# tencent-ailab/V-Express

Hardware: AMD Instinct MI355X
Metric: decoded frames/sec at 512x512, 25 DDIM steps (higher is better)
Workload: dtype bf16; 1 GPU; 512x512, 16 frames (1 window(s) of 16, overlap 4), 25 DDIM steps, CFG 3.5, random-init UNet3D + ReferenceNet banks + sd-vae-ft-mse decode; frames=16, windows=1, parallelism=window x CFG-half units over 1 GPU(s)

## Files before the change

### v-express_amd/csrc/vx_attn.hip

```cpp
#include "vx_common.h"
#include <stdio.h>
#include "../../include/vexpress_hip.h"

#include <stdlib.h>

#include <type_traits>

namespace {

struct AttnParams {
  const bf16_t* q; int ldq;
  const bf16_t* k; int ldk;
  const bf16_t* vt; int vt_pitch;
  bf16_t* out; int ldo;
  int batch, heads, n_q, n_kv, d, q_per_kv;
  float c;
  const float* kmax;
};

__device__ __forceinline__ int k_lds_off(int slab, int key, int grp) {
  return slab * 4096 + key * 64 + ((grp ^ ((0 - (key >> 2)) & 3)) << 4);
}
__device__ __forceinline__ int v_lds_off(int row, int chunk) { return row * 128 + ((chunk ^ ((row >> 1) & 7)) << 4); }

// ... 798 lines not shown
    best = fmaxf(best, ss);
  }
  red[threadIdx.x] = best;
  __syncthreads();
  for (int s = 128; s > 0; s >>= 1) {
    if ((int)threadIdx.x < s) red[threadIdx.x] = fmaxf(red[threadIdx.x], red[threadIdx.x + s]);
    __syncthreads();
  }
  if (threadIdx.x == 0) out[bh] = sqrtf(red[0]);
}

constexpr int KNM8_KEYS = 256;
__global__ __launch_bounds__(256) void key_norm_max8_kernel(const bf16_t* __restrict__ k, int ldk, int n_kv, int d,
                                                            float* __restrict__ out) {
  __shared__ float red[4][8];
  const int b = blockIdx.y, key0 = blockIdx.x * KNM8_KEYS;
  const int lane = threadIdx.x & 63, wave = threadIdx.x >> 6, h = lane & 7;
  const bf16_t* base = k + (size_t)b * n_kv * ldk + h * d;
  const int chunks = d >> 3;
  float best = 0.f;
  for (int kk = wave * 8 + (lane >> 3); kk < KNM8_KEYS; kk += 32) {
    const int key = min(key0 + kk, n_kv - 1);
    const bf16_t* row = base + (size_t)key * ldk;
    float ss = 0.f;
    for (int c = 0; c < chunks; ++c) {
      float f[8];
      unpack_bf16x8(*reinterpret_cast<const uint4*>(row + 8 * c), f);
#pragma unroll
      for (int e = 0; e < 8; ++e) ss = fmaf(f[e], f[e], ss);
    }
    best = fmaxf(best, ss);
  }
  best = fmaxf(best, __shfl_xor(best, 8, 64));
  best = fmaxf(best, __shfl_xor(best, 16, 64));
  best = fmaxf(best, __shfl_xor(best, 32, 64));
  if (lane < 8) red[wave][lane] = best;
  __syncthreads();
  if (threadIdx.x < 8) {
    const float m = fmaxf(fmaxf(red[0][threadIdx.x], red[1][threadIdx.x]), fmaxf(red[2][threadIdx.x], red[3][threadIdx.x]));
    atomicMax(reinterpret_cast<unsigned int*>(out) + b * 8 + threadIdx.x, __float_as_uint(sqrtf(m)));
  }
}

int attention_impl(const void* q, int ldq, const void* k, int ldk, const void* vt, int vt_pitch, void* out, int ldo,
                   int batch, int heads, int n_q, int n_kv, int head_dim, int q_per_kv, float scale,
                   const float* key_norm_max, hipStream_t stream);

}

int vx_attn3_variant();
int vx_attn3_launch(const void* q, int ldq, const void* k, int ldk, const void* vt, int vt_pitch, void* out, int ldo,
                    int batch, int heads, int n_q, int n_kv, int q_per_kv, float c, const float* kmax,
                    hipStream_t stream);

extern "C" int vx_key_norm_max(const void* k, int ldk, int kv_batches, int heads, int n_kv, int head_dim, float* out,
                               void* stream) {
  VX_REQUIRE(k && out, "vx_key_norm_max: null pointer");
  VX_REQUIRE(kv_batches > 0 && heads > 0 && n_kv > 0 && head_dim > 0 && (head_dim % 8) == 0 && (ldk % 8) == 0,
             "vx_key_norm_max: bad sizes (head_dim=%d ldk=%d)", head_dim, ldk);
  static int v8 = -1;
  if (v8 < 0) {
    const char* e = getenv("VX_KNM8");
    v8 = !(e && atoi(e) == 0);
  }
  if (v8 && heads == 8 && n_kv >= 2 * KNM8_KEYS && kv_batches <= 65535) {
    if (hipMemsetAsync(out, 0, (size_t)kv_batches * heads * sizeof(float), (hipStream_t)stream) != hipSuccess) {
      vx_set_error("vx_key_norm_max: hipMemsetAsync failed");
      return VX_ERR_HIP;
    }
    hipLaunchKernelGGL(key_norm_max8_kernel, dim3((n_kv + KNM8_KEYS - 1) / KNM8_KEYS, kv_batches), dim3(256), 0,
                       (hipStream_t)stream, (const bf16_t*)k, ldk, n_kv, head_dim, out);
    return vx_check_launch("vx_key_norm_max");
  }
  hipLaunchKernelGGL(key_norm_max_kernel, dim3(kv_batches * heads), dim3(256), 0, (hipStream_t)stream,
                     (const bf16_t*)k, ldk, heads, n_kv, head_dim, out);
  return vx_check_launch("vx_key_norm_max");
}

extern "C" int vx_attention(const void* q, int ldq, const void* k, int ldk, const void* vt, int vt_pitch, void* out,
                            int ldo, int batch, int heads, int n_q, int n_kv, int head_dim, int q_per_kv,
                            float scale, void* stream) {
  return attention_impl(q, ldq, k, ldk, vt, vt_pitch, out, ldo, batch, heads, n_q, n_kv, head_dim, q_per_kv, scale,
                        nullptr, (hipStream_t)stream);
}

extern "C" int vx_attention_bounded(const void* q, int ldq, const void* k, int ldk, const void* vt, int vt_pitch,
                                    void* out, int ldo, int batch, int heads, int n_q, int n_kv, int head_dim,
                                    int q_per_kv, float scale, const float* key_norm_max, void* stream) {
  VX_REQUIRE(key_norm_max != nullptr, "vx_attention_bounded: null key_norm_max");
  return attention_impl(q, ldq, k, ldk, vt, vt_pitch, out, ldo, batch, heads, n_q, n_kv, head_dim, q_per_kv, scale,
                        key_norm_max, (hipStream_t)stream);
}

namespace {
int attention_impl(const void* q, int ldq, const void* k, int ldk, const void* vt, int vt_pitch, void* out, int ldo,
                   int batch, int heads, int n_q, int n_kv, int head_dim, int q_per_kv, float scale,
                   const float* key_norm_max, hipStream_t stream) {
  VX_REQUIRE(q && k && vt && out, "vx_attention: null pointer");
  VX_REQUIRE(batch > 0 && heads > 0 && n_q > 0 && n_kv > 0 && q_per_kv > 0 && (batch % q_per_kv) == 0,
             "vx_attention: bad sizes");
  VX_REQUIRE((head_dim % 8) == 0 && (ldq % 8) == 0 && (ldk % 8) == 0 && (vt_pitch % 8) == 0 && (ldo % 4) == 0 &&
                 vt_pitch >= n_kv,
             "vx_attention: alignment (head_dim=%d ldq=%d ldk=%d pitch=%d ldo=%d)", head_dim, ldq, ldk, vt_pitch, ldo);
  VX_REQUIRE((long)batch * heads <= 65535, "vx_attention: batch*heads too large for grid.y");
  AttnParams p{(const bf16_t*)q, ldq, (const bf16_t*)k, ldk, (const bf16_t*)vt, vt_pitch, (bf16_t*)out, ldo,
               batch, heads, n_q, n_kv, head_dim, q_per_kv, scale == 0.f ? 1.0f : scale * 1.4426950408889634f,
               key_norm_max};
  VX_REQUIRE(scale >= 0.f, "vx_attention: scale must be positive (or 0: K carries scale * log2 e)");
  const int d = head_dim;
  static int v1 = -1;
  if (v1 < 0) v1 = getenv("VX_ATTN_V1") != nullptr;
  if (!v1 && d == 40 && key_norm_max && vx_attn3_variant() > 0 && ((size_t)n_kv * ldk * 2) < (1ull << 31) &&
      ((size_t)d * vt_pitch * 2) < (1ull << 31))
    return vx_attn3_launch(q, ldq, k, ldk, vt, vt_pitch, out, ldo, batch, heads, n_q, n_kv, q_per_kv, p.c, key_norm_max,
                           stream);
  if (!v1 && d > 32 && d <= 48 && (d % 16) != 0)
    return key_norm_max ? launch_attn2<2, 3, 2, true, true>(p, stream) : launch_attn2<2, 3, 2, true, false>(p, stream);
  if (d <= 32) return launch_attn<1, 2, 4, true>(p, stream);
  if (d <= 48) return launch_attn<2, 3, 2, true>(p, stream);
  if (d <= 64) return launch_attn<2, 4, 2, true>(p, stream);
  if (d <= 80) return launch_attn<3, 5, 2, true>(p, stream);
  if (d <= 96) return launch_attn<3, 6, 2, true>(p, stream);
  if (d <= 128) return launch_attn<4, 8, 2, true>(p, stream);
  if (d <= 160) return launch_attn<5, 10, 2, false>(p, stream);
  if (d == 512) return launch_attn<16, 32, 1, false, 1>(p, stream);
  vx_set_error("vx_attention: unsupported head_dim %d", d);
  return VX_ERR_UNSUPPORTED;
}
}

extern "C" int vx_temporal_attention(const void* qkv, int ldqkv, void* out, int ldo, int b, int f, int hw, int heads,
                                     int head_dim, float scale, void* stream_) {
  hipStream_t stream = (hipStream_t)stream_;
  VX_REQUIRE(qkv && out, "vx_temporal_attention: null pointer");
  VX_REQUIRE(f >= 1 && f <= 32, "vx_temporal_attention: f=%d outside [1,32] (PositionalEncoding max_len)", f);
  VX_REQUIRE((head_dim % 8) == 0 && (ldqkv % 8) == 0 && (ldo % 4) == 0, "vx_temporal_attention: alignment");
  TemporalParams p{(const bf16_t*)qkv, ldqkv, (bf16_t*)out, ldo, b, f, hw, heads, head_dim,
                   scale * 1.4426950408889634f};
  const int d = head_dim;
  if (d <= 32) return launch_temporal<1, 2>(p, stream);
  if (d <= 64) return launch_temporal<2, 4>(p, stream);
  if (d <= 96) return launch_temporal<3, 6>(p, stream);
  if (d <= 128) return launch_temporal<4, 8>(p, stream);
  if (d <= 160) return launch_temporal<5, 10>(p, stream);
  vx_set_error("vx_temporal_attention: unsupported head_dim %d", d);
  return VX_ERR_UNSUPPORTED;
}

extern "C" int vx_small_kv_attention(const void* q, int ldq, const void* kv, int ldkv, int v_off, void* out, int ldo,
                                     int batch, int n_q, int n_kv, int heads, int head_dim, float scale,
                                     void* stream_) {
  hipStream_t stream = (hipStream_t)stream_;
  VX_REQUIRE(q && kv && out, "vx_small_kv_attention: null pointer");
  VX_REQUIRE(n_kv >= 1 && n_kv <= SKV_MAX, "vx_small_kv_attention: n_kv=%d outside [1,%d]", n_kv, SKV_MAX);
  VX_REQUIRE((head_dim % 8) == 0 && (ldq % 8) == 0 && (ldkv % 8) == 0 && (v_off % 8) == 0 && (ldo % 8) == 0,
             "vx_small_kv_attention: alignment");
  const int C = heads * head_dim;
  size_t smem = (size_t)n_kv * 2 * C * sizeof(bf16_t);
  VX_REQUIRE(smem <= 64 * 1024, "vx_small_kv_attention: K/V tile %zu B exceeds LDS budget", smem);
  dim3 grid(ceil_div((long)n_q * heads, 256), batch);
  hipLaunchKernelGGL(small_kv_attn_kernel, grid, dim3(256), smem, stream, (const bf16_t*)q, ldq, (const bf16_t*)kv,
                     ldkv, v_off, (bf16_t*)out, ldo, n_q, n_kv, heads, head_dim, scale * 1.4426950408889634f);
  return vx_check_launch("vx_small_kv_attention");
}
```

### v-express_amd/ops.py

```python
import ctypes as C
import logging
import os

import torch

from . import lib as L

class _CurrentLib:

    def __getattr__(self, name):
        return getattr(L.current(), name)


_lib = _CurrentLib()


def __getattr__(name):
    if name == "BF16":
        return L.ELEM[0]
    raise AttributeError(name)


def _stream():
    return C.c_void_p(torch.cuda.current_stream().cuda_stream)
# ... 805 lines not shown
    if not GN_FOLD[0] or t is None or hw % RING_BM or n % RING_BN or c % 64:
        return _note_path("groupnorm_proj_in", geom, False, applied, "fold off or geometry not whole 256 x 320 tiles per frame")
    if _ring_off(c):
        return _note_path("groupnorm_proj_in", geom, False, applied, "persistent kernel switched off")
    ok = t[1] >= RING_MIN_TILES and n * 2 <= hw
    return _note_path("groupnorm_proj_in", geom, ok, folded if ok else applied,
                      "" if ok else "per-frame weight copies would cost more than the normalised tensor")


def groupnorm_stats(x1, *, frames, hw, groups, x2=None):
    _chk_bf16(x1, "x1")
    st = gn_of(x1) if x2 is None else None
    if st is not None and st.fits(frames, hw, groups, x1.shape[-1]):
        return st.ws, st.slabs
    if not x1.is_contiguous() or (x2 is not None and not x2.is_contiguous()):
        raise ValueError("groupnorm inputs must be contiguous")
    c1 = x1.shape[-1]
    c2 = x2.shape[-1] if x2 is not None else 0
    slices = _gn_slices(hw)
    ws = torch.empty(int(_lib.vx_groupnorm_ws_floats(frames, slices, groups)), device=x1.device, dtype=torch.float32)
    with _hbm_op("groupnorm_stats", 2 * frames * hw * (c1 + c2)):
        L.check(_lib.vx_groupnorm_stats(_ptr(x1), c1, _ptr(x2), c2, frames, hw, groups, _ptr(ws), slices, _stream()),
                "vx_groupnorm_stats")
    return ws, slices


def groupnorm_fold_linear(ws, gamma, w, bias_beta, *, frames, hw, groups, eps, slices=None):
    _chk_bf16(w, "w")
    n, c = w.shape
    if bias_beta.dtype != torch.float32 or gamma.dtype != torch.float32 or not w.is_contiguous():
        raise TypeError("groupnorm_fold_linear: float32 gamma / bias_beta, contiguous bf16 weight expected")
    w_f = torch.empty((frames, n, c), device=w.device, dtype=L.ELEM[0])
    b_f = torch.empty((frames, n), device=w.device, dtype=torch.float32)
    L.check(_lib.vx_groupnorm_fold_linear(_ptr(ws), frames, hw, slices or _gn_slices(hw), groups, float(eps), _ptr(gamma), c,
                                          _ptr(w), _ptr(bias_beta), n, _ptr(w_f), _ptr(b_f), _stream()),
            "vx_groupnorm_fold_linear")
    return w_f, b_f


def layernorm(x, gamma, beta, eps=1e-5, *, add=None, add_rows_per_entry=1, add_entries=1, out=None):
    _chk_bf16(x, "x")
    ldx, rows = _row_stride(x)
    c = x.shape[-1]
    if out is None:
        out = torch.empty((rows, c), device=x.device, dtype=L.ELEM[0])
    with _hbm_op("layernorm", 4 * rows * c):
        L.check(_lib.vx_layernorm(_ptr(x), ldx, rows, c, float(eps), _ptr(gamma), _ptr(beta), _ptr(add),
                                  add_rows_per_entry, add_entries, _ptr(out), _row_stride(out)[0], _stream()),
                "vx_layernorm")
    return out


_BOUNDED_SOFTMAX = [os.environ.get("VX_ATTN_BOUND", "1") != "0"]


def key_norm_max(k, *, kv_batches, heads, n_kv, head_dim):
    ldk, _ = _row_stride(k)
    out = torch.empty((kv_batches * heads,), device=k.device, dtype=torch.float32)
    with _hbm_op("key_norm_max", 2 * kv_batches * n_kv * heads * head_dim):
        L.check(_lib.vx_key_norm_max(_ptr(k), ldk, kv_batches, heads, n_kv, head_dim, _ptr(out), _stream()),
                "vx_key_norm_max")
    return out


def attention(q, k, vt, *, batch, heads, n_q, n_kv, head_dim, q_per_kv=1, out=None, kmax=None, k_prescaled=False):
    ldq, _ = _row_stride(q)
    ldk, _ = _row_stride(k)
    if out is None:
        out = torch.empty((batch * n_q, heads * head_dim), device=q.device, dtype=L.ELEM[0])
    scale = 0.0 if k_prescaled else head_dim ** -0.5
    c = heads * head_dim
    flops = 4.0 * batch * heads * n_q * n_kv * head_dim
    nbytes = 2 * (2 * batch * n_q * c + 2 * (batch // q_per_kv) * n_kv * c)
    if _BOUNDED_SOFTMAX[0] and 32 < head_dim <= 48 and head_dim % 16:
        if kmax is None:
            kmax = key_norm_max(k, kv_batches=batch // q_per_kv, heads=heads, n_kv=n_kv, head_dim=head_dim)
        with _hbm_op("attention", nbytes, flops=flops):
            L.check(_lib.vx_attention_bounded(_ptr(q), ldq, _ptr(k), ldk, _ptr(vt), vt.shape[-1], _ptr(out),
                                              _row_stride(out)[0], batch, heads, n_q, n_kv, head_dim, q_per_kv,
                                              scale, _ptr(kmax), _stream()), "vx_attention_bounded")
        return out
    with _hbm_op("attention", nbytes, flops=flops):
        L.check(_lib.vx_attention(_ptr(q), ldq, _ptr(k), ldk, _ptr(vt), vt.shape[-1], _ptr(out), _row_stride(out)[0],
                                  batch, heads, n_q, n_kv, head_dim, q_per_kv, scale, _stream()),
                "vx_attention")
    return out


def temporal_attention(qkv, *, b, f, hw, heads, head_dim, out=None):
    _chk_bf16(qkv, "qkv")
    ld, rows = _row_stride(qkv)
    if rows != b * f * hw:
        raise ValueError("qkv rows != b*f*hw")
    if out is None:
        out = torch.empty((rows, heads * head_dim), device=qkv.device, dtype=L.ELEM[0])
    with _hbm_op("temporal_attention", 2 * rows * 4 * heads * head_dim, flops=4.0 * rows * f * heads * head_dim):
        L.check(_lib.vx_temporal_attention(_ptr(qkv), ld, _ptr(out), _row_stride(out)[0], b, f, hw, heads, head_dim,
                                           head_dim ** -0.5, _stream()), "vx_temporal_attention")
    return out


def small_kv_attention(q, kv, *, batch, n_q, n_kv, heads, head_dim, out=None):
    ldq, _ = _row_stride(q)
    ldkv, _ = _row_stride(kv)
    c = heads * head_dim
    if out is None:
        out = torch.empty((batch * n_q, c), device=q.device, dtype=L.ELEM[0])
    with _hbm_op("small_kv_attention", 2 * (2 * batch * n_q * c + 2 * batch * n_kv * c)):
        L.check(_lib.vx_small_kv_attention(_ptr(q), ldq, _ptr(kv), ldkv, c, _ptr(out), _row_stride(out)[0], batch, n_q,
                                           n_kv, heads, head_dim, head_dim ** -0.5, _stream()),
                "vx_small_kv_attention")
    return out


UPSAMPLE_PHASES = [os.environ.get("VX_UPSAMPLE_PHASES", "1") != "0"]
UPSAMPLE_PHASES_MIN_HW = [int(os.environ.get("VX_UPSAMPLE_PHASES_MIN_HW", "256"))]


def upsample_phases_applies(H, W, c):
    geom = (("hw_in", H * W), ("c", c))
    four, one = "four 2x2 convolutions over the original image + interleave", "one 3x3 convolution with the upsampling in its gather"
    ok = UPSAMPLE_PHASES[0] and H * W >= UPSAMPLE_PHASES_MIN_HW[0] and c % 64 == 0
    return _note_path("upsample_conv", geom, ok, four if ok else one,
                      "" if ok else "switched off / input frame below VX_UPSAMPLE_PHASES_MIN_HW pixels / channels not a multiple of 64")


def pad_image(x, frames, H, W):
# ... 350 lines not shown
```

### v-express_amd/csrc/vx_norm.hip

```cpp
#include "vx_common.h"
#include "vx_gemm_common.h"
#include "../../include/vexpress_hip.h"

namespace {

constexpr int GN_THREADS = 256;
constexpr int GN_MAX_SETS = 2;

constexpr int GN_UNROLL = 4;
constexpr int GN_SUBS = 8;

struct GnPlan {
  const bf16_t* base[GN_MAX_SETS];
  int pstride[GN_MAX_SETS];
  int chunk[GN_MAX_SETS];
  int pl, pl_count;
};

__device__ __forceinline__ GnPlan gn_plan(const bf16_t* x1, int c1, const bf16_t* x2, int c2, int hw, int frame) {
  GnPlan P;
  const int nchunks = (c1 + c2) >> 3;
  const int tid = threadIdx.x;
  const int tp = nchunks < GN_THREADS ? nchunks : GN_THREADS;
  P.pl_count = GN_THREADS / tp;
// ... 207 lines not shown
    shift[ch] = beta[ch] - gstat[g * 2 + 0] * sc;
  }
  __syncthreads();
  const GnPlan P = gn_plan(x1, c1, x2, c2, hw, frame);
  const int p_begin = slice * slice_pix;
  const int p_end = min(hw, p_begin + slice_pix);
  const int wp = width + 2 * out_pad;
  const int hp = hw / width + 2 * out_pad;
  bf16_t* const oframe = out + (size_t)frame * hp * wp * C;
  auto opix = [&](int px) {
    if (out_pad == 0) return px;
    const int y = w_shift >= 0 ? px >> w_shift : px / width;
    return (y + out_pad) * wp + (px - y * width) + out_pad;
  };
#pragma unroll
  for (int u = 0; u < GN_MAX_SETS; ++u) {
    if (P.base[u] == nullptr) continue;
    const bf16_t* src = P.base[u];
    const int ps = P.pstride[u];
    const int ch = P.chunk[u] * 8;
    float sc[8], sh[8];
#pragma unroll
    for (int e = 0; e < 8; ++e) {
      sc[e] = scale[ch + e];
      sh[e] = shift[ch + e];
    }
    auto emit = [&](const uint4& raw, int px) {
      float f[8];
      unpack_bf16x8(raw, f);
#pragma unroll
      for (int e = 0; e < 8; ++e) f[e] = f[e] * sc[e] + sh[e];
      if (silu == 1) {
#pragma unroll
        for (int e = 0; e < 8; ++e) f[e] = silu_f(f[e]);
      } else if (silu == 2) {
#pragma unroll
        for (int e = 0; e < 8; ++e) f[e] = gelu_f(f[e]);
      }
      *reinterpret_cast<uint4*>(oframe + (size_t)opix(px) * C + ch) = pack_bf16x8(f);
    };
    int px = p_begin + P.pl;
    for (; px + (GN_UNROLL - 1) * P.pl_count < p_end; px += GN_UNROLL * P.pl_count) {
      uint4 raw[GN_UNROLL];
#pragma unroll
      for (int k = 0; k < GN_UNROLL; ++k)
        raw[k] = *reinterpret_cast<const uint4*>(src + (size_t)(px + k * P.pl_count) * ps);
#pragma unroll
      for (int k = 0; k < GN_UNROLL; ++k) emit(raw[k], px + k * P.pl_count);
    }
    for (; px < p_end; px += P.pl_count) emit(*reinterpret_cast<const uint4*>(src + (size_t)px * ps), px);
  }
}

constexpr int LN_R = 4;

template <int MAXC>
__global__ __launch_bounds__(256) void layernorm_kernel(const bf16_t* __restrict__ x, int ldx, int rows, int c,
                                                        float eps, const float* __restrict__ gamma,
                                                        const float* __restrict__ beta,
                                                        const float* __restrict__ add, int add_rows_per_entry,
                                                        int add_entries, bf16_t* __restrict__ out, int ldo) {
  const int lane = threadIdx.x & 63;
  const int wave = blockIdx.x * 4 + (threadIdx.x >> 6);
  const int nwaves = gridDim.x * 4;
  const int nchunks = c >> 3;
  const float inv_c = 1.0f / (float)c;
  bool live[MAXC];
  float g[MAXC][8], b[MAXC][8];
#pragma unroll
  for (int u = 0; u < MAXC; ++u) {
    const int chunk = lane + u * 64;
    live[u] = chunk < nchunks;
    const int cs = live[u] ? chunk : 0;
    const float4 g0 = *reinterpret_cast<const float4*>(gamma + cs * 8);
    const float4 g1 = *reinterpret_cast<const float4*>(gamma + cs * 8 + 4);
    const float4 b0 = *reinterpret_cast<const float4*>(beta + cs * 8);
    const float4 b1 = *reinterpret_cast<const float4*>(beta + cs * 8 + 4);
    g[u][0] = g0.x; g[u][1] = g0.y; g[u][2] = g0.z; g[u][3] = g0.w;
    g[u][4] = g1.x; g[u][5] = g1.y; g[u][6] = g1.z; g[u][7] = g1.w;
    b[u][0] = b0.x; b[u][1] = b0.y; b[u][2] = b0.z; b[u][3] = b0.w;
    b[u][4] = b1.x; b[u][5] = b1.y; b[u][6] = b1.z; b[u][7] = b1.w;
  }
  for (int row0 = wave * LN_R; row0 < rows; row0 += nwaves * LN_R) {
    uint4 raw[LN_R][MAXC];
#pragma unroll
    for (int r = 0; r < LN_R; ++r) {
      const int row = min(row0 + r, rows - 1);
#pragma unroll
      for (int u = 0; u < MAXC; ++u) {
        const int chunk = live[u] ? lane + u * 64 : 0;
        raw[r][u] = *reinterpret_cast<const uint4*>(x + (size_t)row * ldx + chunk * 8);
      }
    }
    float sum[LN_R];
#pragma unroll
    for (int r = 0; r < LN_R; ++r) {
      sum[r] = 0.f;
#pragma unroll
      for (int u = 0; u < MAXC; ++u) {
        float v[8];
        unpack_bf16x8(raw[r][u], v);
        float t = ((v[0] + v[1]) + (v[2] + v[3])) + ((v[4] + v[5]) + (v[6] + v[7]));
        sum[r] += live[u] ? t : 0.f;
      }
    }
#pragma unroll
// ... 153 lines not shown
      float sq = 0.f;
#pragma unroll
      for (int u = 0; u < MAXC; ++u) {
        if (lane + u * 64 < nchunks) {
#pragma unroll
          for (int e = 0; e < 8; ++e) {
            const float d = y[u][e] - mean;
            sq += d * d;
          }
        }
      }
#pragma unroll
      for (int m = 32; m >= 1; m >>= 1) sq = wave_xor_sum(sq, m);
      const float rstd = rsqrtf(sq * inv_c + eps);
      const float* addrow = add != nullptr ? add + (size_t)((row / add_rows_per_entry) % add_entries) * c : nullptr;
#pragma unroll
      for (int u = 0; u < MAXC; ++u) {
        const int chunk = lane + u * 64;
        if (chunk < nchunks) {
#pragma unroll
          for (int e = 0; e < 8; ++e) {
            float o = (y[u][e] - mean) * rstd * gamma[chunk * 8 + e] + beta[chunk * 8 + e];
            if (addrow != nullptr) o += addrow[chunk * 8 + e];
            y[u][e] = o;
          }
        }
      }
    }
    float amax = 0.f;
#pragma unroll
    for (int u = 0; u < MAXC; ++u)
#pragma unroll
      for (int e = 0; e < 8; ++e) amax = fmaxf(amax, fabsf(y[u][e]));
#pragma unroll
    for (int m = 32; m >= 1; m >>= 1) amax = wave_xor_max(amax, m);
    const float sc = amax > 0.f ? amax * (1.0f / 448.0f) : 1.0f;
    const float inv = 1.0f / sc;
    if (lane == 0) scale[row] = sc;
#pragma unroll
    for (int u = 0; u < MAXC; ++u) {
      const int chunk = lane + u * 64;
      if (chunk < ochunks) {
        int w0 = 0, w1 = 0;
        w0 = __builtin_amdgcn_cvt_pk_fp8_f32(y[u][0] * inv, y[u][1] * inv, w0, false);
        w0 = __builtin_amdgcn_cvt_pk_fp8_f32(y[u][2] * inv, y[u][3] * inv, w0, true);
        w1 = __builtin_amdgcn_cvt_pk_fp8_f32(y[u][4] * inv, y[u][5] * inv, w1, false);
        w1 = __builtin_amdgcn_cvt_pk_fp8_f32(y[u][6] * inv, y[u][7] * inv, w1, true);
        *reinterpret_cast<uint2*>(out8 + (size_t)row * ldo8 + chunk * 8) = make_uint2((uint32_t)w0, (uint32_t)w1);
      }
    }
  }
}

}

extern "C" int64_t vx_groupnorm_ws_floats(int frames, int slices, int groups) {
  return (int64_t)frames * slices * groups * 2;
}

extern "C" int vx_groupnorm(const void* x1, int c1, const void* x2, int c2, int frames, int hw, int groups, float eps,
                            const float* gamma, const float* beta, int silu, void* out, float* ws, int slices,
                            int width, int out_pad, void* stream_) {
  hipStream_t stream = (hipStream_t)stream_;
  const int C = c1 + c2;
  VX_REQUIRE(x1 != nullptr && out != nullptr && ws != nullptr && gamma != nullptr && beta != nullptr,
             "vx_groupnorm: null pointer");
  VX_REQUIRE((c2 == 0) == (x2 == nullptr), "vx_groupnorm: x2/c2 mismatch");
  VX_REQUIRE(c1 > 0 && (c1 % 8) == 0 && (c2 % 8) == 0, "vx_groupnorm: channels must be multiples of 8");
  VX_REQUIRE(groups > 0 && (C % groups) == 0, "vx_groupnorm: C=%d not divisible by groups=%d", C, groups);
  VX_REQUIRE(C <= 8 * GN_THREADS * GN_MAX_SETS, "vx_groupnorm: C=%d too large", C);
  VX_REQUIRE(frames > 0 && hw > 0 && slices > 0 && slices <= hw, "vx_groupnorm: bad geometry");
  VX_REQUIRE(silu >= 0 && silu <= 2, "vx_groupnorm: activation code %d (0 none, 1 SiLU, 2 erf-GELU)", silu);
  VX_REQUIRE(out_pad >= 0 && (out_pad == 0 || (width > 0 && hw % width == 0)),
             "vx_groupnorm: padded output needs the image width (hw=%d width=%d)", hw, width);
  if (out_pad == 0) width = hw;
  int w_shift = -1;
  for (int sft = 0; sft < 31; ++sft)
    if ((1 << sft) == width) w_shift = sft;
  const int slice_pix = ceil_div(hw, slices);
  const int nchunks = C / 8;
  const int tp = nchunks < GN_THREADS ? nchunks : GN_THREADS;
  const int pl_count = GN_THREADS / tp;
  size_t smem_stats = (size_t)pl_count * C * 2 * sizeof(float);
  size_t smem_apply = (size_t)(2 * C + 2 * groups) * sizeof(float) + (size_t)GN_SUBS * groups * 2 * sizeof(double);
  VX_REQUIRE(smem_stats <= 64 * 1024, "vx_groupnorm: stats LDS %zu too large", smem_stats);
  hipLaunchKernelGGL(gn_stats_kernel, dim3(frames * slices), dim3(GN_THREADS), smem_stats, stream,
                     (const bf16_t*)x1, c1, (const bf16_t*)x2, c2, hw, groups, slices, slice_pix, ws);
  int rc = vx_check_launch("vx_groupnorm(stats)");
  if (rc) return rc;
  static int amax = -1;
  if (amax < 0) {
    const char* e = getenv("VX_GN_APPLY_SLICES");
    amax = e ? atoi(e) : 64;
    if (amax < 1) amax = 1;
  }
  const int aslices = slices < amax ? slices : amax;
  const int apix = ceil_div(hw, aslices);
  hipLaunchKernelGGL(gn_apply_kernel, dim3(frames * aslices), dim3(GN_THREADS), smem_apply, stream,
                     (const bf16_t*)x1, c1, (const bf16_t*)x2, c2, hw, groups, eps, gamma, beta, silu,
                     (bf16_t*)out, aslices, apix, (const float*)ws, width, w_shift, out_pad, slices);
  return vx_check_launch("vx_groupnorm(apply)");
}

extern "C" int vx_groupnorm_apply(const void* x1, int c1, const void* x2, int c2, int frames, int hw, int groups,
                                  float eps, const float* gamma, const float* beta, int silu, void* out,
                                  const float* ws, int stat_slices, int slices, int width, int out_pad, void* stream_) {
  hipStream_t stream = (hipStream_t)stream_;
  const int C = c1 + c2;
  VX_REQUIRE(x1 != nullptr && out != nullptr && ws != nullptr && gamma != nullptr && beta != nullptr,
             "vx_groupnorm_apply: null pointer");
  VX_REQUIRE((c2 == 0) == (x2 == nullptr), "vx_groupnorm_apply: x2/c2 mismatch");
  VX_REQUIRE(c1 > 0 && (c1 % 8) == 0 && (c2 % 8) == 0, "vx_groupnorm_apply: channels must be multiples of 8");
  VX_REQUIRE(groups > 0 && (C % groups) == 0, "vx_groupnorm_apply: C=%d not divisible by groups=%d", C, groups);
  VX_REQUIRE(C <= 8 * GN_THREADS * GN_MAX_SETS, "vx_groupnorm_apply: C=%d too large", C);
  VX_REQUIRE(frames > 0 && hw > 0 && slices > 0 && slices <= hw && stat_slices > 0, "vx_groupnorm_apply: bad geometry");
  VX_REQUIRE(silu >= 0 && silu <= 2, "vx_groupnorm_apply: activation code %d (0 none, 1 SiLU, 2 erf-GELU)", silu);
  VX_REQUIRE(out_pad >= 0 && (out_pad == 0 || (width > 0 && hw % width == 0)),
             "vx_groupnorm_apply: padded output needs the image width (hw=%d width=%d)", hw, width);
  if (out_pad == 0) width = hw;
  int w_shift = -1;
  for (int sft = 0; sft < 31; ++sft)
    if ((1 << sft) == width) w_shift = sft;
  const size_t smem_apply = (size_t)(2 * C + 2 * groups) * sizeof(float) + (size_t)GN_SUBS * groups * 2 * sizeof(double);
  const int apix = ceil_div(hw, slices);
  hipLaunchKernelGGL(gn_apply_kernel, dim3(frames * slices), dim3(GN_THREADS), smem_apply, stream, (const bf16_t*)x1, c1,
                     (const bf16_t*)x2, c2, hw, groups, eps, gamma, beta, silu, (bf16_t*)out, slices, apix, ws, width,
                     w_shift, out_pad, stat_slices);
  return vx_check_launch("vx_groupnorm_apply");
}

extern "C" int vx_groupnorm_stats(const void* x1, int c1, const void* x2, int c2, int frames, int hw, int groups,
// ... 172 lines not shown
```

Baseline: 14.12 frames/s.

## Add bounded-softmax single-pass attention kernel for head_dim 80

Adds a dedicated attention kernel for head_dim 80. It uses a precomputed key-norm bound (|q|·max|k|) as a fixed softmax shift, so the online max/rescale work disappears. The row sum is folded into an extra MFMA column of ones, and K/V tiles are double-buffered through direct global-to-LDS loads. Python routing now computes key_norm_max and calls the bounded entry for d=80 when n_q>=128. If the row sums underflow, the kernel falls back to a max pass plus a recompute, and the extra key_norm_max launch adds overhead.

```diff
diff --git a/v-express_amd/csrc/vx_attn.hip b/v-express_amd/csrc/vx_attn.hip
--- a/v-express_amd/csrc/vx_attn.hip
+++ b/v-express_amd/csrc/vx_attn.hip
@@ -874,6 +874,10 @@
 int vx_attn3_launch(const void* q, int ldq, const void* k, int ldk, const void* vt, int vt_pitch, void* out, int ldo,
                     int batch, int heads, int n_q, int n_kv, int q_per_kv, float c, const float* kmax,
                     hipStream_t stream);
+bool vx_attn80_enabled();
+int vx_attn80_launch(const void* q, int ldq, const void* k, int ldk, const void* vt, int vt_pitch, void* out, int ldo,
+                     int batch, int heads, int n_q, int n_kv, int q_per_kv, float c, const float* kmax,
+                     hipStream_t stream);
 
 extern "C" int vx_key_norm_max(const void* k, int ldk, int kv_batches, int heads, int n_kv, int head_dim, float* out,
                                void* stream) {
@@ -936,6 +940,10 @@
       ((size_t)d * vt_pitch * 2) < (1ull << 31))
     return vx_attn3_launch(q, ldq, k, ldk, vt, vt_pitch, out, ldo, batch, heads, n_q, n_kv, q_per_kv, p.c, key_norm_max,
                            stream);
+  if (!v1 && d == 80 && key_norm_max && n_q >= 128 && vx_attn80_enabled() && ((size_t)n_kv * ldk * 2) < (1ull << 31) &&
+      ((size_t)d * vt_pitch * 2) < (1ull << 31))
+    return vx_attn80_launch(q, ldq, k, ldk, vt, vt_pitch, out, ldo, batch, heads, n_q, n_kv, q_per_kv, p.c, key_norm_max,
+                            stream);
   if (!v1 && d > 32 && d <= 48 && (d % 16) != 0)
     return key_norm_max ? launch_attn2<2, 3, 2, true, true>(p, stream) : launch_attn2<2, 3, 2, true, false>(p, stream);
   if (d <= 32) return launch_attn<1, 2, 4, true>(p, stream);
diff --git a/v-express_amd/csrc/vx_attn80.hip b/v-express_amd/csrc/vx_attn80.hip
--- /dev/null
+++ b/v-express_amd/csrc/vx_attn80.hip
@@ -0,0 +1,306 @@
+#include "vx_common.h"
+#include "vx_gemm_common.h"
+
+#include <stdlib.h>
+
+#include <type_traits>
+
+namespace {
+
+struct Attn80Params {
+  const bf16_t* q; int ldq;
+  const bf16_t* k; int ldk;
+  const bf16_t* vt; int vt_pitch;
+  bf16_t* out; int ldo;
+  int batch, heads, n_q, n_kv, q_per_kv;
+  float c;
+  const float* kmax;
+};
+
+constexpr int A8_D = 80;
+constexpr int A8_KA = 0;
+constexpr int A8_KB = 4096;
+constexpr int A8_KC = 8192;
+constexpr int A8_V = 10240;
+constexpr int A8_STAGE = A8_V + 96 * 128;
+constexpr int A8_NBUF = 2;
+constexpr int A8_QT = 2;
+constexpr int A8_PIECES = 5;
+constexpr int A8_ONES = A8_NBUF * A8_STAGE, A8_ZERO = A8_ONES + 1024;
+constexpr int A8_SMEM = A8_ZERO + 1024;
+
+__device__ __forceinline__ int a8_pi(int r) { return 32 * (r >> 5) + 8 * ((r >> 2) & 3) + 4 * ((r >> 4) & 1) + (r & 3); }
+
+template <bool UNIT>
+__global__ __launch_bounds__(256, 3) void attn80_kernel(const Attn80Params p) {
+  extern __shared__ __attribute__((aligned(16))) char smem[];
+  const int tid = threadIdx.x, lane = tid & 63;
+  const int wave = __builtin_amdgcn_readfirstlane(tid >> 6);
+  const int i = lane & 15, g = lane >> 4;
+  const int nqb = (p.n_q + 64 * A8_QT - 1) / (64 * A8_QT);
+  const int lid = xcd_remap(blockIdx.x, gridDim.x);
+  const int bh = lid / nqb, qb = lid - bh * nqb;
+  const int b = bh / p.heads, h = bh - b * p.heads;
+  const int kvb = b / p.q_per_kv;
+  const int q0 = qb * (64 * A8_QT) + wave * (16 * A8_QT);
+  const bf16_t* __restrict__ kbase = p.k + (size_t)kvb * p.n_kv * p.ldk + h * A8_D;
+  const bf16_t* __restrict__ vbase = p.vt + (size_t)(kvb * p.heads + h) * A8_D * p.vt_pitch;
+  const int n_tiles = (p.n_kv + 63) >> 6;
+  const bool ragged = (p.n_kv & 63) != 0;
+
+  for (int idx = tid; idx < 128; idx += 256) {
+    *reinterpret_cast<uint4*>(smem + A8_ONES + idx * 16) = idx < 64 ? make_uint4(VX_E16_ONE, 0, 0, 0) : make_uint4(0, 0, 0, 0);
+  }
+  for (int idx = tid; idx < A8_NBUF * 128; idx += 256) {
+    const int st = idx >> 7, r = 80 + ((idx >> 3) & 15), j = idx & 7;
+    *reinterpret_cast<uint4*>(smem + st * A8_STAGE + A8_V + r * 128 + j * 16) =
+        r == 80 ? make_uint4(VX_E16_ONE2, VX_E16_ONE2, VX_E16_ONE2, VX_E16_ONE2) : make_uint4(0, 0, 0, 0);
+  }
+
+  const uint32_t kstep = 128u * (uint32_t)p.ldk, vstep = 128u;
+  auto src_of = [&](int s, int l, int te) -> uint32_t {
+    const int pw = wave + 4 * s;
+    if (pw < 10) {
+      int r, chunk;
+      if (pw < 8) {
+        r = 16 * (pw & 3) + (l >> 2);
+        chunk = 4 * (pw >> 2) + ((l & 3) ^ ((0 - (r >> 2)) & 3));
+      } else {
+        r = 32 * (pw - 8) + (l >> 1);
+        chunk = 8 + (l & 1);
+      }
+      uint32_t off = ((uint32_t)a8_pi(r) * (uint32_t)p.ldk + 8u * chunk) * 2u;
+      if (te >= 0) {
+        const int over = te * 64 + a8_pi(r) - (p.n_kv - 1);
+        off += (uint32_t)te * kstep - (over > 0 ? (uint32_t)over * (uint32_t)p.ldk * 2u : 0u);
+      }
+      return off;
+    }
+    const int r = 8 * (pw - 10) + (l >> 3), chunk = (l & 7) ^ ((r >> 1) & 7);
+    uint32_t off = ((uint32_t)r * (uint32_t)p.vt_pitch + 8u * chunk) * 2u;
+    if (te >= 0) off += (uint32_t)te * vstep - (te * 64 + 8 * chunk >= p.n_kv ? 16u * chunk : 0u);
+    return off;
+  };
+  uint32_t src0[A8_PIECES];
+#pragma unroll
+  for (int s = 0; s < A8_PIECES; ++s) src0[s] = src_of(s, lane, -1);
+  const uint32_t lds0 = lds_addr_of(smem);
+  auto issue = [&](int t) {
+    const uint32_t so = lds0 + (uint32_t)(t % A8_NBUF) * A8_STAGE;
+    if (ragged && t == n_tiles - 1) {
+      int l = lane;
+      asm volatile("" : "+v"(l));
+#pragma unroll
+      for (int s = 0; s < A8_PIECES; ++s) {
+        const bool is_k = wave + 4 * s < 10;
+        glds16_s(is_k ? (const void*)kbase : (const void*)vbase, src_of(s, l, t), so + 1024u * (uint32_t)(wave + 4 * s));
+      }
+      return;
+    }
+#pragma unroll
+    for (int s = 0; s < A8_PIECES; ++s) {
+      const bool is_k = wave + 4 * s < 10;
+      glds16_s(is_k ? (const void*)kbase : (const void*)vbase, src0[s] + (uint32_t)t * (is_k ? kstep : vstep),
+               so + 1024u * (uint32_t)(wave + 4 * s));
+    }
+  };
+
+  uint4 qf[A8_QT][3];
+  float mfix[A8_QT];
+#pragma unroll
+  for (int qt = 0; qt < A8_QT; ++qt) {
+    const int qrow = q0 + 16 * qt + i;
+    float ss = 0.f;
+#pragma unroll
+    for (int kk = 0; kk < 3; ++kk) {
+      const int dcol = 32 * kk + 8 * g;
+      uint4 v = make_uint4(0, 0, 0, 0);
+      if (qrow < p.n_q && dcol < A8_D) {
+        v = *reinterpret_cast<const uint4*>(p.q + (size_t)(b * p.n_q + qrow) * p.ldq + h * A8_D + dcol);
+        float f[8];
+        unpack_bf16x8(v, f);
+#pragma unroll
+        for (int e = 0; e < 8; ++e) ss = fmaf(f[e], f[e], ss);
+      }
+      qf[qt][kk] = v;
+    }
+    ss = wave_xor_sum(ss, 16);
+    ss = wave_xor_sum(ss, 32);
+    mfix[qt] = sqrtf(ss) * p.kmax[kvb * p.heads + h] - (UNIT ? VX_P_HEADROOM : VX_P_HEADROOM / p.c);
+  }
+  auto set_shift = [&](const float (&m)[A8_QT]) {
+#pragma unroll
+    for (int qt = 0; qt < A8_QT; ++qt)
+      if (g == 2) qf[qt][2] = make_uint4((uint32_t)f32_to_bf16(-m[qt]), 0, 0, 0);
+  };
+
+  const int ksw = (g ^ ((0 - (i >> 2)) & 3)) << 4;
+  const int a_ka = A8_KA + i * 64 + ksw;
+  const int a_kb = A8_KB + i * 64 + ksw;
+  const int a_kc = g < 2 ? A8_KC + i * 32 + g * 16 : (g == 2 ? A8_ONES : A8_ZERO) + i * 16;
+  const int kc_step = g < 2 ? 512 : 256;
+  const int kc_stage = g < 2 ? 1 : 0;
+  const int vx = (i >> 1) & 7;
+  const int a_v0 = A8_V + i * 128 + ((g ^ vx) << 4);
+  const int a_v1 = A8_V + i * 128 + (((4 | g) ^ vx) << 4);
+
+  f32x4_t o[6][A8_QT];
+  auto zero_o = [&]() {
+#pragma unroll
+    for (int qt = 0; qt < A8_QT; ++qt)
+#pragma unroll
+      for (int dt = 0; dt < 6; ++dt) o[dt][qt] = f32x4_t{0.f, 0.f, 0.f, 0.f};
+  };
+
+  auto qk = [&](f32x4_t (&s_)[4][A8_QT], int t) {
+    const int so = (t % A8_NBUF) * A8_STAGE;
+    const char* ka = smem + a_ka + so;
+    const char* kb = smem + a_kb + so;
+    const char* kc = smem + a_kc + so * kc_stage;
+#pragma unroll
+    for (int kt = 0; kt < 4; ++kt) {
+      const uint4 kf0 = *reinterpret_cast<const uint4*>(ka + kt * 1024);
+      const uint4 kf1 = *reinterpret_cast<const uint4*>(kb + kt * 1024);
+      const uint4 kf2 = *reinterpret_cast<const uint4*>(kc + kt * kc_step);
+#pragma unroll
+      for (int qt = 0; qt < A8_QT; ++qt) {
+        s_[kt][qt] = mfma16(kf0, qf[qt][0], f32x4_t{0.f, 0.f, 0.f, 0.f});
+        s_[kt][qt] = mfma16(kf1, qf[qt][1], s_[kt][qt]);
+        s_[kt][qt] = mfma16(kf2, qf[qt][2], s_[kt][qt]);
+      }
+    }
+  };
+  auto mask = [&](f32x4_t (&s_)[4][A8_QT], int t) {
+#pragma unroll
+    for (int kt = 0; kt < 4; ++kt)
+#pragma unroll
+      for (int r = 0; r < 4; ++r)
+        if (t * 64 + 32 * (kt >> 1) + 8 * g + 4 * (kt & 1) + r >= p.n_kv) {
+#pragma unroll
+          for (int qt = 0; qt < A8_QT; ++qt) s_[kt][qt][r] = -INFINITY;
+        }
+  };
+  auto expo = [&](f32x4_t (&s_)[4][A8_QT]) {
+#pragma unroll
+    for (int kt = 0; kt < 4; ++kt)
+#pragma unroll
+      for (int qt = 0; qt < A8_QT; ++qt)
+#pragma unroll
+        for (int r = 0; r < 4; ++r) s_[kt][qt][r] = __builtin_amdgcn_exp2f(UNIT ? s_[kt][qt][r] : s_[kt][qt][r] * p.c);
+  };
+  auto pv = [&](const f32x4_t (&s_)[4][A8_QT], int t) {
+    const int so = (t % A8_NBUF) * A8_STAGE;
+#pragma unroll
+    for (int ks_ = 0; ks_ < 2; ++ks_) {
+      uint4 pb[A8_QT];
+#pragma unroll
+      for (int qt = 0; qt < A8_QT; ++qt) {
+        const f32x4_t& a = s_[2 * ks_][qt];
+        const f32x4_t& c2 = s_[2 * ks_ + 1][qt];
+        pb[qt] = make_uint4(pack_bf16x2(a[0], a[1]), pack_bf16x2(a[2], a[3]), pack_bf16x2(c2[0], c2[1]),
+                            pack_bf16x2(c2[2], c2[3]));
+      }
+      const char* vp = smem + (ks_ ? a_v1 : a_v0) + so;
+#pragma unroll
+      for (int dt = 0; dt < 6; ++dt) {
+        const uint4 vf = *reinterpret_cast<const uint4*>(vp + dt * 2048);
+#pragma unroll
+        for (int qt = 0; qt < A8_QT; ++qt) o[dt][qt] = mfma16(vf, pb[qt], o[dt][qt]);
+      }
+    }
+  };
+
+  float mrun[A8_QT];
+  auto run = [&](auto maxpass_c) {
+    constexpr bool MAXPASS = decltype(maxpass_c)::value;
+    __syncthreads();
+    issue(0);
+    for (int t = 0; t < n_tiles; ++t) {
+      asm volatile("s_waitcnt vmcnt(0)" ::: "memory");
+      __syncthreads();
+      if (t + 1 < n_tiles) issue(t + 1);
+      f32x4_t cur[4][A8_QT];
+      qk(cur, t);
+      if (ragged && t == n_tiles - 1) mask(cur, t);
+      if (MAXPASS) {
+#pragma unroll
+        for (int qt = 0; qt < A8_QT; ++qt) {
+          float mx = mrun[qt];
+#pragma unroll
+          for (int kt = 0; kt < 4; ++kt)
+            mx = fmaxf(fmaxf(fmaxf(mx, cur[kt][qt][0]), fmaxf(cur[kt][qt][1], cur[kt][qt][2])), cur[kt][qt][3]);
+          mrun[qt] = mx;
+        }
+      } else {
+        expo(cur);
+        pv(cur, t);
+      }
+    }
+  };
+  auto row_sum = [&](int qt) -> float { return __shfl(o[5][qt][0], i, 64); };
+
+  set_shift(mfix);
+  zero_o();
+  run(std::false_type{});
+  bool bad = false;
+#pragma unroll
+  for (int qt = 0; qt < A8_QT; ++qt) {
+    const float l = row_sum(qt);
+    bad |= (q0 + 16 * qt + i < p.n_q) && !(l >= VX_P_MIN_ROWSUM(p.n_kv));
+  }
+  if (__syncthreads_or(bad)) {
+    const float zero[A8_QT] = {0.f, 0.f};
+    set_shift(zero);
+#pragma unroll
+    for (int qt = 0; qt < A8_QT; ++qt) mrun[qt] = -INFINITY;
+    run(std::true_type{});
+#pragma unroll
+    for (int qt = 0; qt < A8_QT; ++qt) mrun[qt] = wave_rows_max(mrun[qt]);
+    set_shift(mrun);
+    zero_o();
+    run(std::false_type{});
+  }
+
+#pragma unroll
+  for (int qt = 0; qt < A8_QT; ++qt) {
+    const float inv = 1.0f / row_sum(qt);
+    const int qrow = q0 + 16 * qt + i;
+    if (qrow >= p.n_q) continue;
+    bf16_t* orow = p.out + (size_t)(b * p.n_q + qrow) * p.ldo + h * A8_D;
+#pragma unroll
+    for (int dt = 0; dt < 5; ++dt) {
+      uint2 w;
+      w.x = pack_bf16x2(o[dt][qt][0] * inv, o[dt][qt][1] * inv);
+      w.y = pack_bf16x2(o[dt][qt][2] * inv, o[dt][qt][3] * inv);
+      *reinterpret_cast<uint2*>(orow + 16 * dt + 4 * g) = w;
+    }
+  }
+}
+
+template <bool UNIT>
+int launch_attn80(const Attn80Params& p, hipStream_t stream) {
+  auto kern = attn80_kernel<UNIT>;
+  dim3 grid((unsigned)((long)ceil_div(p.n_q, 64 * A8_QT) * p.batch * p.heads));
+  g_vx_last_kernel = UNIT ? "attn80_kernel<true>" : "attn80_kernel<false>";
+  hipLaunchKernelGGL(kern, grid, dim3(256), A8_SMEM, stream, p);
+  return vx_check_launch("vx_attention");
+}
+
+}
+
+bool vx_attn80_enabled() {
+  static int v = -1;
+  if (v < 0) {
+    const char* e = getenv("VX_ATTN80");
+    v = !(e && atoi(e) == 0);
+  }
+  return v != 0;
+}
+
+int vx_attn80_launch(const void* q, int ldq, const void* k, int ldk, const void* vt, int vt_pitch, void* out, int ldo,
+                     int batch, int heads, int n_q, int n_kv, int q_per_kv, float c, const float* kmax,
+                     hipStream_t stream) {
+  Attn80Params p{(const bf16_t*)q, ldq, (const bf16_t*)k, ldk, (const bf16_t*)vt, vt_pitch, (bf16_t*)out, ldo,
+                 batch, heads, n_q, n_kv, q_per_kv, c, kmax};
+  return c == 1.0f ? launch_attn80<true>(p, stream) : launch_attn80<false>(p, stream);
+}
diff --git a/v-express_amd/ops.py b/v-express_amd/ops.py
--- a/v-express_amd/ops.py
+++ b/v-express_amd/ops.py
@@ -881,6 +881,7 @@
 
 
 _BOUNDED_SOFTMAX = [os.environ.get("VX_ATTN_BOUND", "1") != "0"]
+_ATTN80 = os.environ.get("VX_ATTN80", "1").strip() not in ("0", "")
 
 
 def key_norm_max(k, *, kv_batches, heads, n_kv, head_dim):
@@ -901,7 +902,7 @@
     c = heads * head_dim
     flops = 4.0 * batch * heads * n_q * n_kv * head_dim
     nbytes = 2 * (2 * batch * n_q * c + 2 * (batch // q_per_kv) * n_kv * c)
-    if _BOUNDED_SOFTMAX[0] and 32 < head_dim <= 48 and head_dim % 16:
+    if _BOUNDED_SOFTMAX[0] and ((32 < head_dim <= 48 and head_dim % 16) or (_ATTN80 and head_dim == 80 and n_q >= 128)):
         if kmax is None:
             kmax = key_norm_max(k, kv_batches=batch // q_per_kv, heads=heads, n_kv=n_kv, head_dim=head_dim)
         with _hbm_op("attention", nbytes, flops=flops):
```

Result: no change. 14.20 frames/s (median of 6 runs) (+0.6%).

## Add single-pass register-resident GroupNorm kernel replacing stats+apply launches

Applied to the files above, without the earlier changes.

Adds a one-pass GroupNorm kernel where each block owns a frame and a slab of groups and keeps all its pixels in registers. It computes the mean and then a centered variance through block reductions in shared memory, and applies the affine transform plus SiLU/GELU with optional padded output. This replaces the two-kernel stats/apply path and its global workspace round-trip whenever the plan fits, which is at most 16 chunks per thread. The cost is high register pressure and fewer blocks for large hw or few groups, which could hurt occupancy.

```diff
diff --git a/v-express_amd/csrc/vx_norm.hip b/v-express_amd/csrc/vx_norm.hip
--- a/v-express_amd/csrc/vx_norm.hip
+++ b/v-express_amd/csrc/vx_norm.hip
@@ -283,6 +283,152 @@
   }
 }
 
+constexpr int GN1_MAX_GSLAB = 8;
+__device__ __forceinline__ void gn_keep_packed(uint4& r) { asm volatile("" : "+v"(r.x), "+v"(r.y), "+v"(r.z), "+v"(r.w)); }
+
+template <int NT, int NCH>
+__global__ __launch_bounds__(NT) void gn_onepass_kernel(const bf16_t* __restrict__ x1, int c1,
+                                                        const bf16_t* __restrict__ x2, int c2, int hw, int groups,
+                                                        float eps, const float* __restrict__ gamma,
+                                                        const float* __restrict__ beta, int silu,
+                                                        bf16_t* __restrict__ out, int kchunks, int gslab, int width,
+                                                        int w_shift, int out_pad) {
+  __shared__ float part[NT * 2];
+  __shared__ float gst[GN1_MAX_GSLAB * 2];
+  const int C = c1 + c2, cg = C / groups;
+  const int nslabs = groups / gslab;
+  const int bid = VX_XCD_ROWS ? xcd_remap(blockIdx.x, gridDim.x) : (int)blockIdx.x;
+  const int frame = bid / nslabs, slab = bid % nslabs;
+  const int tid = threadIdx.x, lane = tid & 63, wave = tid >> 6;
+  const int K = kchunks, PL = NT / K;
+  const int kc = tid % K, pl = tid / K;
+  const bool active = pl < PL;
+  const int rel = kc * 8;
+  const int ch = slab * gslab * cg + rel;
+  const int glo = rel / cg;
+  const int ghi = (rel + 7) / cg;
+  const int split = (glo + 1) * cg - rel;
+  const bf16_t* src;
+  int ps;
+  if (ch < c1) {
+    src = x1 + (size_t)frame * hw * c1 + ch;
+    ps = c1;
+  } else {
+    src = x2 + (size_t)frame * hw * c2 + (ch - c1);
+    ps = c2;
+  }
+  uint4 raw[NCH];
+#pragma unroll
+  for (int j = 0; j < NCH; ++j) raw[j] = *reinterpret_cast<const uint4*>(src + (size_t)min(pl + j * PL, hw - 1) * ps);
+
+  auto block_sums = [&](float lo, float hi, int slot) {
+    if (active) *reinterpret_cast<float2*>(part + (pl * K + kc) * 2) = make_float2(lo, hi);
+    __syncthreads();
+    for (int g = wave; g < gslab; g += NT / 64) {
+      const int kfirst = (g * cg) >> 3, nk = (((g + 1) * cg - 1) >> 3) - kfirst + 1;
+      float a = 0.f;
+      for (int idx = lane; idx < PL * nk; idx += 64) {
+        const int p = idx / nk, k = kfirst + (idx - p * nk);
+        a += part[(p * K + k) * 2 + ((k * 8) / cg == g ? 0 : 1)];
+      }
+#pragma unroll
+      for (int m = 32; m >= 1; m >>= 1) a = wave_xor_sum(a, m);
+      if (lane == 0) {
+        const float v = a / ((float)cg * (float)hw);
+        gst[g * 2 + slot] = slot == 0 ? v : 1.0f / sqrtf(v + eps);
+      }
+    }
+    __syncthreads();
+  };
+
+  float s[8];
+#pragma unroll
+  for (int e = 0; e < 8; ++e) s[e] = 0.f;
+#pragma unroll
+  for (int j = 0; j < NCH; ++j) {
+    const bool live = active && pl + j * PL < hw;
+    float f[8];
+    unpack_bf16x8(raw[j], f);
+#pragma unroll
+    for (int e = 0; e < 8; ++e) s[e] += live ? f[e] : 0.f;
+  }
+  float lo = 0.f, hi = 0.f;
+#pragma unroll
+  for (int e = 0; e < 8; ++e) {
+    if (e < split) lo += s[e];
+    else hi += s[e];
+  }
+  block_sums(lo, hi, 0);
+
+  const float4 g0 = *reinterpret_cast<const float4*>(gamma + ch), g1 = *reinterpret_cast<const float4*>(gamma + ch + 4);
+  const float4 b0 = *reinterpret_cast<const float4*>(beta + ch), b1 = *reinterpret_cast<const float4*>(beta + ch + 4);
+  float mean[8];
+  {
+    const float mlo = gst[glo * 2], mhi = gst[ghi * 2];
+#pragma unroll
+    for (int e = 0; e < 8; ++e) mean[e] = e < split ? mlo : mhi;
+  }
+#pragma unroll
+  for (int e = 0; e < 8; ++e) s[e] = 0.f;
+#pragma unroll
+  for (int j = 0; j < NCH; ++j) {
+    const bool live = active && pl + j * PL < hw;
+    float f[8];
+    gn_keep_packed(raw[j]);
+    unpack_bf16x8(raw[j], f);
+#pragma unroll
+    for (int e = 0; e < 8; ++e) {
+      const float d = f[e] - mean[e];
+      s[e] += live ? d * d : 0.f;
+    }
+  }
+  lo = hi = 0.f;
+#pragma unroll
+  for (int e = 0; e < 8; ++e) {
+    if (e < split) lo += s[e];
+    else hi += s[e];
+  }
+  block_sums(lo, hi, 1);
+
+  float sc[8], sh[8];
+  {
+    const float rlo = gst[glo * 2 + 1], rhi = gst[ghi * 2 + 1];
+    const float ga[8] = {g0.x, g0.y, g0.z, g0.w, g1.x, g1.y, g1.z, g1.w};
+    const float be[8] = {b0.x, b0.y, b0.z, b0.w, b1.x, b1.y, b1.z, b1.w};
+#pragma unroll
+    for (int e = 0; e < 8; ++e) {
+      sc[e] = ga[e] * (e < split ? rlo : rhi);
+      sh[e] = be[e] - mean[e] * sc[e];
+    }
+  }
+  const int wp = width + 2 * out_pad;
+  const int hp = hw / width + 2 * out_pad;
+  bf16_t* const dst = out + (size_t)frame * hp * wp * C + ch;
+#pragma unroll
+  for (int j = 0; j < NCH; ++j) {
+    const int px = pl + j * PL;
+    if (!active || px >= hw) continue;
+    float f[8];
+    gn_keep_packed(raw[j]);
+    unpack_bf16x8(raw[j], f);
+#pragma unroll
+    for (int e = 0; e < 8; ++e) f[e] = f[e] * sc[e] + sh[e];
+    if (silu == 1) {
+#pragma unroll
+      for (int e = 0; e < 8; ++e) f[e] = silu_f(f[e]);
+    } else if (silu == 2) {
+#pragma unroll
+      for (int e = 0; e < 8; ++e) f[e] = gelu_f(f[e]);
+    }
+    int op = px;
+    if (out_pad != 0) {
+      const int y = w_shift >= 0 ? px >> w_shift : px / width;
+      op = (y + out_pad) * wp + (px - y * width) + out_pad;
+    }
+    *reinterpret_cast<uint4*>(dst + (size_t)op * C) = pack_bf16x8(f);
+  }
+}
+
 constexpr int LN_R = 4;
 
 template <int MAXC>
@@ -542,6 +688,33 @@
   }
 }
 
+}
+
+struct GnOnePass {
+  int gslab, kchunks, threads, nch;
+};
+static bool gn_onepass_plan(int hw, int C, int groups, GnOnePass* P) {
+  static int on = -1;
+  if (on < 0) {
+    const char* e = getenv("VX_GN_ONEPASS");
+    on = (e && atoi(e) == 0) ? 0 : 1;
+  }
+  const int cg = C / groups;
+  if (!on || cg < 8) return false;
+  int g = 1;
+  while (g <= GN1_MAX_GSLAB && (g * cg) % 8 != 0) g *= 2;
+  while (g * cg * 2 < 128 && g * 2 <= GN1_MAX_GSLAB && groups % (g * 2) == 0) g *= 2;
+  if (g > GN1_MAX_GSLAB || groups % g != 0) return false;
+  const int k = g * cg / 8;
+  if (k > 256) return false;
+  for (int nt = 256; nt <= 1024; nt *= 4) {
+    const int need = ceil_div(hw, nt / k);
+    if (need <= 16) {
+      *P = GnOnePass{g, k, nt, nt == 256 && need <= 4 ? 4 : 16};
+      return true;
+    }
+  }
+  return false;
 }
 
 extern "C" int64_t vx_groupnorm_ws_floats(int frames, int slices, int groups) {
@@ -567,6 +740,23 @@
   int w_shift = -1;
   for (int sft = 0; sft < 31; ++sft)
     if ((1 << sft) == width) w_shift = sft;
+  GnOnePass op;
+  if (gn_onepass_plan(hw, C, groups, &op)) {
+    const dim3 grid(frames * (groups / op.gslab));
+#define VX_GN1(NT, NCH, SYM)                                                                                            \
+  do {                                                                                                                  \
+    hipLaunchKernelGGL((gn_onepass_kernel<NT, NCH>), grid, dim3(NT), 0, stream, (const bf16_t*)x1, c1,                  \
+                       (const bf16_t*)x2, c2, hw, groups, eps, gamma, beta, silu, (bf16_t*)out, op.kchunks, op.gslab,   \
+                       width, w_shift, out_pad);                                                                        \
+    g_vx_last_kernel = SYM;                                                                                             \
+  } while (0)
+    if (op.threads == 1024) VX_GN1(1024, 16, "gn_onepass_kernel<1024, 16>");
+    else if (op.nch == 4) VX_GN1(256, 4, "gn_onepass_kernel<256, 4>");
+    else VX_GN1(256, 16, "gn_onepass_kernel<256, 16>");
+#undef VX_GN1
+    return vx_check_launch("vx_groupnorm(one pass)");
+  }
+  g_vx_last_kernel = "gn_stats_kernel + gn_apply_kernel";
   const int slice_pix = ceil_div(hw, slices);
   const int nchunks = C / 8;
   const int tp = nchunks < GN_THREADS ? nchunks : GN_THREADS;
```

New measurement: 13.94 frames/s before, 13.97 frames/s after, median of 5. Within noise of the previous version (+0.2%).
